# EvolEcolGroup/tidypopgen

Measured on AMD Instinct MI355X. Metric: SNP-genotypes/s (N x M) for IBS+KING+GRM+Fst+PCA; max |delta| vs CPU ref (cpu_baseline.parity), higher is better.
Workload: dtype fp4-e2m1 operands (exact integers, f32 accumulate) for the cross-products, the PCA Gram and the grouped counts, int8 (int32 accumulate) for the loadings, f64 for statistics

## Files before the change

### tidypopgen_amd/csrc/pca.hip

```cpp
#include <math.h>
#include <stdio.h>
#include <stdlib.h>
#include <string.h>
#include <time.h>

#include <algorithm>

#include "common.h"
#include <type_traits>
#include "devfrag.h"

#define MFMA_I8(a, b, c) __builtin_amdgcn_mfma_i32_32x32x32_i8((a), (b), (c), 0, 0, 0)
#define PCA_NAN __longlong_as_double(0x7FF8000000000000ll)

__global__ void tpg_pca_center_scale_kernel(const int4* __restrict__ counts, int64_t m, int64_t n,
                                            double* __restrict__ center, double* __restrict__ scale,
                                            int* __restrict__ flags) {
  for (int64_t j = blockIdx.x * (int64_t)blockDim.x + threadIdx.x; j < m; j += (int64_t)gridDim.x * blockDim.x) {
    const int4 c = counts[j];
    if (c.w != 0) flags[0] = 1;
    const double mean = (double)(c.y + 2 * c.z) / (double)n;
    const double p = mean / 2;
    const double sd = sqrt(2 * p * (1 - p));
    if (!(sd > 0)) flags[1] = 1;
// ... 1225 lines not shown
    std::vector<double> RR;
    if (first) {
      lam1 = fabs(theta[0]) > 0 ? fabs(theta[0]) : 1.0;
    } else {
      TPG_TRY(w.ritz(A, Y, act, X, theta, Y0, Y1, RR));
      TPG_HIP(tpg_copy_dev(ctx, A, Y0, colbytes(act)));
      if (nl == 0) lam1 = fabs(theta[0]) > 0 ? fabs(theta[0]) : 1.0;
      st.mark("ritz vectors + residuals");
    }
    int newly = 0;
    while (!first && newly < act && nl + newly < k && sqrt(std::max(0.0, RR[(size_t)newly])) < TOL * lam1) newly++;
    for (int j = 0; j < newly; j++) lam[(size_t)(nl + j)] = theta[(size_t)j];
    nl += newly;
    if (nl >= k) break;
    const int act2 = b - nl;
    TPG_REQUIRE(act2 >= 2, TPG_ENUMERIC, "eigen solver ran out of active vectors");
    double* A2 = Q + (size_t)n * nl;
    const double* KA2 = first ? Y : Y1 + (size_t)n * newly;
    const double up = std::max(theta[(size_t)act - 1], 1e-300 * lam1), lo = 0.0;
    const double a0 = std::max(theta[(size_t)newly], up * (1 + 1e-8));
    const double ec = (up - lo) / 2, cc = (up + lo) / 2;
    const double x0 = (a0 - cc) / ec;
    int deg = 20;
    if (x0 > 1.0 + 1e-12) {
      const double dmax = log(2 * AMP) / acosh(x0);
      deg = dmax < 2 ? 2 : (dmax > 20 ? 20 : (int)dmax);
    }
    if (tpg_env_set("TPG_DEBUG"))
      fprintf(stderr, "[eig] it %d act %d locked %d (+%d) deg %d theta_first %.4g theta_last %.4g lam1 %.4g res0 %.3g\n", it,
              act, nl, newly, deg, theta[(size_t)newly], theta[(size_t)act - 1], lam1,
              first ? -1.0 : sqrt(std::max(0.0, RR[(size_t)newly])) / lam1);
    w.b = act2;
    TPG_TRY(w.set_locked(Q, nl, lam.data()));
    double sigma = ec / (a0 - cc);
    const double sigma1 = sigma;
    double* prev = Y0;
    double* cur = first ? Y1 : Y;
    double* nxt = first ? Y : Y1;
    TPG_HIP(tpg_copy_dev(ctx, prev, A2, colbytes(act2)));
    TPG_LAUNCH(ctx, "eig_combine", tpg_combine_kernel, dim3(1024), dim3(256), 0, KA2, 1, (int64_t)n * act2,
               sigma1 / ec, (const double*)prev, -cc * sigma1 / ec, (const double*)nullptr, 0.0, cur,
               (const double*)nullptr);
    for (int dgr = 2; dgr <= deg; dgr++) {
      const double sigma2 = 1.0 / (2.0 / sigma1 - sigma);
      TPG_TRY(w.apply(cur, 2 * sigma2 / ec, cur, -2 * sigma2 * cc / ec, prev, -sigma * sigma2, nxt));
      double* t = prev; prev = cur; cur = nxt; nxt = t;
      sigma = sigma2;
    }
    TPG_HIP(tpg_copy_dev(ctx, A2, cur, colbytes(act2)));
    st.mark("chebyshev filter");
    TPG_TRY(orthonormalize(A2, act2, Q, nl, prev));
    st.mark("orthonormalize");
  }
  TPG_REQUIRE(nl >= k, TPG_ENUMERIC, "eigen solver did not converge (%d of %d pairs)", nl, k);
  for (int j = 0; j < k; j++) lambda_host[j] = lam[(size_t)j];
  TPG_HIP(tpg_copy_dev(ctx, d_U, Q, colbytes(k)));
  return TPG_OK;
}

static int pca_loadings_device(tpg_ctx* ctx, const tpg_view* v, const double* d_center, const double* d_scale,
                               const double* d_U, const double* d_dk, int k, double* d_V);

__global__ __launch_bounds__(256) void tpg_deflate_kernel(double* __restrict__ K, int n, const double* __restrict__ U,
                                                          const double* __restrict__ lam, int kb) {
  __shared__ double ui[16][33], uj[16][33];
  const int tx = threadIdx.x & 15, ty = threadIdx.x >> 4;
  const int i0 = blockIdx.x * 16, j0 = blockIdx.y * 16;
  for (int q = threadIdx.x; q < 16 * kb; q += 256) {
    const int r = q & 15, c = q >> 4;
    ui[r][c] = i0 + r < n ? U[(int64_t)(i0 + r) + (int64_t)c * n] * lam[c] : 0.0;
    uj[r][c] = j0 + r < n ? U[(int64_t)(j0 + r) + (int64_t)c * n] : 0.0;
  }
  __syncthreads();
  const int i = i0 + tx, j = j0 + ty;
  if (i >= n || j >= n) return;
  double s = 0.0;
  for (int c = 0; c < kb; c++) s = fma(ui[tx][c], uj[ty][c], s);
  K[(int64_t)i + (int64_t)j * n] -= s;
}

static int eig_topk_any(tpg_ctx* ctx, const double* d_K, int n, int k, double* lambda_host, double* d_U, double tol) {
  if (k <= 52) return eig_topk(ctx, d_K, n, k, lambda_host, d_U, tol);
  double *Kw = nullptr, *d_lam = nullptr;
  TPG_HIP(tpg_pmalloc((void**)&Kw, sizeof(double) * (size_t)n * (size_t)n));
  struct Free { void *a, *b; ~Free() { tpg_pfree(a); tpg_pfree(b); } } fr{Kw, nullptr};
  TPG_HIP(tpg_pmalloc((void**)&d_lam, sizeof(double) * 32));
  fr.b = d_lam;
  TPG_HIP(hipMemcpyAsync(Kw, d_K, sizeof(double) * (size_t)n * (size_t)n, hipMemcpyDeviceToDevice, ctx->stream));
  const int KB = 26;
  for (int done = 0; done < k;) {
    const int kb = std::min(KB, k - done);
    double* Ub = d_U + (size_t)done * (size_t)n;
    TPG_TRY(eig_topk(ctx, Kw, n, kb, lambda_host + done, Ub, tol));
    done += kb;
    if (done < k) {
      TPG_HIP(tpg_h2d_async(ctx, d_lam, lambda_host + done - kb, sizeof(double) * (size_t)kb));
      TPG_LAUNCH(ctx, "eig_deflate", tpg_deflate_kernel, dim3((unsigned)((n + 15) / 16), (unsigned)((n + 15) / 16)), dim3(256), 0, Kw, n,
                 (const double*)Ub, (const double*)d_lam, kb);
      TPG_CHECK_LAUNCH();
    }
  }
  return TPG_OK;
}

static int pca_svd_impl(tpg_ctx* ctx, tpg_comm* comm, const tpg_view* v, int k, double tol, double* d, double* u,
                        double* vload, double* center, double* scale, double* square_frobenius);

extern "C" int tpg_pca_partial_svd(tpg_ctx* ctx, const tpg_view* v, int k, double* d, double* u, double* vload,
                                   double* center, double* scale, double* square_frobenius) {
  TpgEnter _enter(ctx);
  return pca_svd_impl(ctx, nullptr, v, k, 1e-12, d, u, vload, center, scale, square_frobenius);
}

extern "C" int tpg_pca_partial_svd_sharded(tpg_ctx* ctx, tpg_comm* comm, const tpg_view* v, int k, double* d, double* u,
                                           double* vload, double* center, double* scale, double* square_frobenius) {
  TpgEnter _enter(ctx);
  TPG_REQUIRE(comm && comm->ctx == ctx, TPG_EINVAL, "bad communicator");
  return pca_svd_impl(ctx, comm, v, k, 1e-12, d, u, vload, center, scale, square_frobenius);
}

extern "C" int tpg_pca_random_svd(tpg_ctx* ctx, const tpg_view* v, int k, double tol, double* d, double* u,
                                  double* vload, double* center, double* scale, double* square_frobenius) {
  TpgEnter _enter(ctx);
  TPG_REQUIRE(tol > 0 && tol < 1, TPG_EINVAL, "tol = %g out of (0, 1)", tol);
  return pca_svd_impl(ctx, nullptr, v, k, tol < 1e-12 ? 1e-12 : tol, d, u, vload, center, scale, square_frobenius);
}

__global__ void tpg_tri_pack_kernel(const double* __restrict__ K, int n, double* __restrict__ tri) {
  const int64_t total = (int64_t)n * n;
  for (int64_t idx = blockIdx.x * (int64_t)blockDim.x + threadIdx.x; idx < total; idx += (int64_t)gridDim.x * blockDim.x) {
    const int64_t i = idx % n, k = idx / n;
    if (i <= k) tri[k * (k + 1) / 2 + i] = K[idx];
  }
}
__global__ void tpg_tri_unpack_kernel(const double* __restrict__ tri, int n, double* __restrict__ K) {
  const int64_t total = (int64_t)n * n;
  for (int64_t idx = blockIdx.x * (int64_t)blockDim.x + threadIdx.x; idx < total; idx += (int64_t)gridDim.x * blockDim.x) {
    const int64_t i = idx % n, k = idx / n;
    const int64_t lo = i < k ? i : k, hi = i < k ? k : i;
    K[idx] = tri[hi * (hi + 1) / 2 + lo];
  }
}

int tpg_pca_gram_allreduce(tpg_ctx* ctx, tpg_comm* comm, double* d_K, int64_t n) {
  if (!comm || !(comm->nranks > 1 || comm->nccl)) return TPG_OK;
  const int64_t ntri = n * (n + 1) / 2;
  double* d_tri = nullptr;
  hipError_t e = tpg_pmalloc((void**)&d_tri, sizeof(double) * (size_t)ntri);
  int lrc = TPG_OK;
  if (e != hipSuccess) { tpg_set_error("gram all-reduce: %s", hipGetErrorString(e)); (void)hipGetLastError(); lrc = TPG_EHIP; }
  lrc = tpg_comm_agree(comm, lrc);
  if (lrc != TPG_OK) { tpg_pfree(d_tri); return lrc; }
  TPG_LAUNCH(ctx, "pca_gram_tri", tpg_tri_pack_kernel, dim3(2048), dim3(256), 0, (const double*)d_K, (int)n, d_tri);
  int rc;
  {
    ProfScope ps(ctx, "pca_gram_allreduce");
    rc = tpg_comm_allreduce(comm, d_tri, ntri, 1);
  }
  if (rc == TPG_OK) TPG_LAUNCH(ctx, "pca_gram_tri", tpg_tri_unpack_kernel, dim3(2048), dim3(256), 0, (const double*)d_tri, (int)n, d_K);
  tpg_pfree(d_tri);
  return rc;
}

static int pca_svd_impl(tpg_ctx* ctx, tpg_comm* comm, const tpg_view* v, int k, double tol, double* d, double* u,
                        double* vload, double* center, double* scale, double* square_frobenius) {
  TPG_REQUIRE(ctx && v && d && u && vload && center && scale, TPG_EINVAL, "null argument");
  TPG_REQUIRE(k >= 1 && k <= v->n, TPG_EINVAL, "k = %d out of range", k);
  const int64_t n = v->n, m = v->m;
  OutBuf oc, os, ou, ov;
  int32_t* d_counts = nullptr;
  double *d_K = nullptr, *d_dk = nullptr, *d_tri = nullptr;
  struct Free { void *a, *b, *c, *d; ~Free() { tpg_pfree(a); tpg_pfree(b); tpg_pfree(c); tpg_pfree(d); } } fr{nullptr, nullptr, nullptr, nullptr};
  StageTimer st(ctx, "svd");
  const bool exchange = comm && (comm->nranks > 1 || comm->nccl);
  const int64_t ntri = n * (n + 1) / 2;
  auto local_steps = [&]() -> int {
    TPG_REQUIRE(k <= m, TPG_EINVAL, "k = %d but this view has %lld loci", k, (long long)m);
    TPG_TRY(oc.init(center, sizeof(double) * (size_t)m));
    TPG_TRY(os.init(scale, sizeof(double) * (size_t)m));
    TPG_TRY(ou.init(u, sizeof(double) * (size_t)n * (size_t)k));
    TPG_TRY(ov.init(vload, sizeof(double) * (size_t)m * (size_t)k));
    TPG_HIP(tpg_pmalloc((void**)&d_counts, sizeof(int32_t) * 4 * (size_t)m));
    fr.a = d_counts;
    TPG_HIP(tpg_pmalloc((void**)&d_K, sizeof(double) * (size_t)n * (size_t)n));
    fr.b = d_K;
    TPG_HIP(tpg_pmalloc((void**)&d_dk, sizeof(double) * (size_t)k));
    fr.d = d_dk;
    if (exchange) {
      TPG_HIP(tpg_pmalloc((void**)&d_tri, sizeof(double) * (size_t)ntri));
      fr.c = d_tri;
    }
    TPG_TRY(pca_counts_center_scale(ctx, v, d_counts, oc.dev<double>(), os.dev<double>()));
    st.mark("counts, center, scale");
    if (square_frobenius) TPG_TRY(frobenius_from_counts(ctx, v, d_counts, oc.dev<double>(), os.dev<double>(), square_frobenius));
    return TPG_OK;
  };
  int lrc = local_steps();
  if (exchange) lrc = tpg_comm_agree(comm, lrc);
  TPG_TRY(lrc);
  if (square_frobenius && exchange) TPG_TRY(tpg_comm_allreduce_f64(ctx, comm, square_frobenius, 1));
  st.mark("frobenius + alloc K");
  auto gram_branch = [&]() -> int {
    bool exchanged = false;
    if (exchange) TPG_TRY(tpg_gram_classes_exchanged(ctx, comm, v, d_counts, os.dev<double>(), d_K, &exchanged));
    if (exchanged) return pca_double_center_inplace(ctx, d_K, n);
    return pca_gram_device(ctx, v, oc.dev<double>(), os.dev<double>(), d_K, true);
  };
  int grc = gram_branch();
  if (exchange) grc = tpg_comm_agree(comm, grc);
  TPG_TRY(grc);
  st.mark("gram");
  if (exchange) {
    TPG_LAUNCH(ctx, "pca_gram_tri", tpg_tri_pack_kernel, dim3(2048), dim3(256), 0, (const double*)d_K, (int)n, d_tri);
    {
      ProfScope ps(ctx, "pca_gram_allreduce");
      TPG_TRY(tpg_comm_allreduce(comm, d_tri, ntri, 1));
    }
    TPG_LAUNCH(ctx, "pca_gram_tri", tpg_tri_unpack_kernel, dim3(2048), dim3(256), 0, (const double*)d_tri, (int)n, d_K);
  }
  std::vector<double> lam((size_t)k);
  TPG_TRY(eig_topk_any(ctx, d_K, (int)n, k, lam.data(), ou.dev<double>(), tol));
  st.mark("eig_topk");
  std::vector<double> dh((size_t)k);
  for (int j = 0; j < k; j++) dh[(size_t)j] = sqrt(lam[(size_t)j] > 0 ? lam[(size_t)j] : 0.0);
  TPG_HIP(tpg_push_small(ctx, d_dk, dh.data(), sizeof(double) * (size_t)k));
  TPG_TRY(pca_loadings_device(ctx, v, oc.dev<double>(), os.dev<double>(), ou.dev<double>(), d_dk, k, ov.dev<double>()));
  if (tpg_is_device_ptr(d)) TPG_HIP(tpg_push_small(ctx, d, dh.data(), sizeof(double) * (size_t)k));
  else memcpy(d, dh.data(), sizeof(double) * (size_t)k);
  TPG_HIP(hipStreamSynchronize(ctx->stream));
  st.mark("loadings");
  TPG_TRY(oc.commit(ctx));
  TPG_TRY(os.commit(ctx));
  TPG_TRY(ou.commit(ctx));
  return ov.commit(ctx);
}

#define LD_TU 6

__global__ void tpg_u_digits_kernel(const double* __restrict__ U, int64_t n, int k, int FU, int64_t Q, int CT,
                                    uint4* __restrict__ UD) {
  const int64_t total = Q * 4 * CT * 64;
  for (int64_t idx = blockIdx.x * (int64_t)blockDim.x + threadIdx.x; idx < total;
       idx += (int64_t)gridDim.x * blockDim.x) {
    const int lane = (int)(idx & 63);
    const int64_t tq = idx >> 6;
    const int ct = (int)(tq % CT);
    const int64_t qs = tq / CT;
    const int s = (int)(qs & 3);
    const int64_t q = qs >> 2;
    const int col = 32 * ct + (lane & 31), h = lane >> 5;
    const int kk = col / LD_TU, t = col % LD_TU;
    uint32_t w[4] = {0, 0, 0, 0};
    if (kk < k)
      for (int e = 0; e < 16; e++) {
        const int64_t i = 128 * q + 32 * s + 16 * h + e;
        if (i >= n) continue;
        long long W = llrint(ldexp(U[i + (int64_t)kk * n], FU));
        long long dig = 0;
        for (int tt = 0; tt <= t; tt++) {
          dig = W & 127;
          if (dig >= 64) dig -= 128;
          W = (W - dig) >> 7;
        }
        w[e >> 2] |= (uint32_t)((int)dig & 0xFF) << (8 * (e & 3));
      }
    UD[idx] = make_uint4(w[0], w[1], w[2], w[3]);
  }
}

__global__ __launch_bounds__(256) void tpg_uq_colsum_kernel(const double* __restrict__ U, int64_t n, int FU,
                                                            double* __restrict__ usum) {
  __shared__ double sh[256];
  const int kk = blockIdx.x;
  double acc = 0;
  for (int64_t i = threadIdx.x; i < n; i += 256) acc += ldexp((double)llrint(ldexp(U[i + (int64_t)kk * n], FU)), -FU);
  sh[threadIdx.x] = acc;
  __syncthreads();
  for (int w = 128; w > 0; w >>= 1) {
    if ((int)threadIdx.x < w) sh[threadIdx.x] += sh[threadIdx.x + w];
    __syncthreads();
  }
  if (threadIdx.x == 0) usum[kk] = sh[0];
}

#ifndef LD_NLT
#define LD_NLT 2
#endif
#ifndef LD_WGS
#define LD_WGS 2
#endif
__device__ __forceinline__ int64_t tpg_uniform64_pca(int64_t x) {
  const uint32_t lo = __builtin_amdgcn_readfirstlane((uint32_t)x), hi = __builtin_amdgcn_readfirstlane((uint32_t)((uint64_t)x >> 32));
  return (int64_t)(((uint64_t)hi << 32) | lo);
}

template <int C, class F>
__device__ __forceinline__ void tpg_pca_static_for(F&& f) {
  if constexpr (C > 0) {
    tpg_pca_static_for<C - 1>(f);
    f(std::integral_constant<int, C - 1>{});
  }
}

template <int CTP>
__global__ __launch_bounds__(256, LD_WGS) void tpg_loadings_mfma_kernel(const uint4* __restrict__ L,
                                                                   const uint4* __restrict__ UD, int64_t n_lt,
                                                                   int64_t Q, int ct0, int CT,
                                                                   int32_t* __restrict__ out, int Cpad) {
  __shared__ __attribute__((aligned(16))) uint4 ubuf[2][4 * CTP][64];
  const int lane = threadIdx.x & 63, wv = threadIdx.x >> 6;
  const int64_t lt0 = ((int64_t)blockIdx.x * 4 + wv) * LD_NLT;
  v16i acc[LD_NLT][CTP];
#pragma unroll
  for (int t = 0; t < LD_NLT; t++)
#pragma unroll
    for (int c = 0; c < CTP; c++)
#pragma unroll
      for (int r = 0; r < 16; r++) acc[t][c][r] = 0;
  const int Qi = (int)Q;
  const int64_t lt0u = tpg_uniform64_pca(lt0);
  const char* pa[LD_NLT];
#pragma unroll
  for (int t = 0; t < LD_NLT; t++) pa[t] = (const char*)(L + ((lt0u + t < n_lt ? lt0u + t : 0) * Q) * 64);
  auto LDG = [&](const char* p, int blk) {
    uint32_t off = (uint32_t)lane * 16u + (uint32_t)blk * 1024u;
    asm("" : "+v"(off));
    return *(const uint4*)(p + off);
  };
  constexpr int LD_D = 4;
  static_assert(LD_D % 2 == 0, "the slot of a group's digit fragments is its parity");
  uint4 AR[LD_D][LD_NLT];
#pragma unroll
  for (int d = 0; d < LD_D - 1; d++)
#pragma unroll
    for (int t = 0; t < LD_NLT; t++) AR[d][t] = LDG(pa[t], d < Qi ? d : Qi - 1);
  const char* pu = (const char*)(UD + ct0 * 64);
  uint4 un[2][CTP];
  auto ufrag = [&](int q, int j) {
    const int it = wv + 4 * j;
    return LDG(pu, (q * 4 + it / CTP) * CT + it % CTP);
  };
#pragma unroll
  for (int j = 0; j < CTP; j++) {
    ubuf[0][wv + 4 * j][lane] = ufrag(0, j);
    un[1][j] = ufrag(Qi > 1 ? 1 : 0, j);
  }
  tpg_lds_barrier();
  auto group = [&](auto Cc, auto Mm, int q) {
    constexpr int C = decltype(Cc)::value, M = decltype(Mm)::value;
    const int qa = q + LD_D - 1 < Qi ? q + LD_D - 1 : Qi - 1, qu = q + 2 < Qi ? q + 2 : Qi - 1;
    const int cur = q & 1;
#pragma unroll
    for (int t = 0; t < LD_NLT; t++) AR[M][t] = LDG(pa[t], qa);
#pragma unroll
    for (int j = 0; j < CTP; j++) un[C & 1][j] = ufrag(qu, j);
#pragma unroll
    for (int s = 0; s < 4; s++) {
      v4i fg[LD_NLT];
#pragma unroll
      for (int t = 0; t < LD_NLT; t++) {
        const uint32_t w = s == 0 ? AR[C][t].x : s == 1 ? AR[C][t].y : s == 2 ? AR[C][t].z : AR[C][t].w;
#pragma unroll
        for (int k = 0; k < 4; k++) fg[t][k] = (int)tpg_codes(w, k);
      }
#pragma unroll
      for (int c = 0; c < CTP; c++) {
        const uint4 bq = ubuf[cur][s * CTP + c][lane];
        v4i fb = {(int)bq.x, (int)bq.y, (int)bq.z, (int)bq.w};
#pragma unroll
        for (int t = 0; t < LD_NLT; t++) acc[t][c] = MFMA_I8(fg[t], fb, acc[t][c]);
      }
    }
#pragma unroll
    for (int j = 0; j < CTP; j++) ubuf[cur ^ 1][wv + 4 * j][lane] = un[(C & 1) ^ 1][j];
    tpg_lds_barrier();
  };
  for (int q = 0; q < Qi; q += LD_D)
    tpg_pca_static_for<LD_D>([&](auto kk) {
      constexpr int k = decltype(kk)::value;
      if (q + k < Qi) group(std::integral_constant<int, k>{}, std::integral_constant<int, (k + LD_D - 1) % LD_D>{}, q + k);
    });
#pragma unroll
  for (int t = 0; t < LD_NLT; t++) {
    if (lt0 + t >= n_lt) break;
#pragma unroll
    for (int c = 0; c < CTP; c++)
#pragma unroll
      for (int r = 0; r < 16; r++) {
        const int64_t row = (lt0 + t) * 32 + tpg_cd_row(r, lane);
        out[row * Cpad + 32 * (ct0 + c) + (lane & 31)] = acc[t][c][r];
      }
  }
}

__global__ void tpg_loadings_finalize_kernel(const int32_t* __restrict__ acc, int Cpad, int64_t m, int k, int FU,
                                             const double* __restrict__ center, const double* __restrict__ scale,
                                             const double* __restrict__ usum, const double* __restrict__ d,
                                             double* __restrict__ vload) {
  const int64_t total = m * k;
  for (int64_t idx = blockIdx.x * (int64_t)blockDim.x + threadIdx.x; idx < total;
       idx += (int64_t)gridDim.x * blockDim.x) {
    const int kk = (int)(idx % k);
    const int64_t j = idx / k;
    long long S = 0;
#pragma unroll
    for (int t = LD_TU - 1; t >= 0; t--) S = S * 128 + (long long)acc[j * Cpad + kk * LD_TU + t];
    const double gu = ldexp((double)S, -FU);
    vload[j + (int64_t)kk * m] = (gu - center[j] * usum[kk]) / (scale[j] * d[kk]);
  }
}

__global__ __launch_bounds__(1024) void tpg_absmax_kernel(const double* __restrict__ x, int64_t total, double* __restrict__ out) {
  __shared__ double sh[1024];
  double mx = 0;
  bool bad = false;
  for (int64_t i = threadIdx.x; i < total; i += 1024) {
    const double a = fabs(x[i]);
    if (a != a) bad = true;
    mx = a > mx ? a : mx;
  }
  sh[threadIdx.x] = bad ? __longlong_as_double(0x7FF8000000000000ll) : mx;
  __syncthreads();
  for (int w = 512; w > 0; w >>= 1) {
    if ((int)threadIdx.x < w) {
      const double a = sh[threadIdx.x], b = sh[threadIdx.x + w];
      sh[threadIdx.x] = (a != a || b != b) ? __longlong_as_double(0x7FF8000000000000ll) : (a > b ? a : b);
    }
    __syncthreads();
  }
  if (threadIdx.x == 0) out[0] = sh[0];
}

static int pca_loadings_device(tpg_ctx* ctx, const tpg_view* v, const double* d_center, const double* d_scale,
                               const double* d_U, const double* d_dk, int k, double* d_V) {
  const int64_t n = v->n, m = v->m;
  double amax = 0;
  {
    double* d_amax = nullptr;
    TPG_HIP(tpg_pmalloc((void**)&d_amax, sizeof(double)));
    TPG_LAUNCH(ctx, "loadings_u_digits", tpg_absmax_kernel, dim3(1), dim3(1024), 0, d_U, n * (int64_t)k, d_amax);
    hipError_t ea = tpg_fetch_small(ctx, &amax, d_amax, sizeof(double));
    tpg_pfree(d_amax);
    TPG_HIP(ea);
  }
  TPG_REQUIRE(amax > 0 && amax == amax && amax < 1e300, TPG_ENUMERIC, "degenerate eigenvectors");
  int ex = 0;
  frexp(amax, &ex);
  const int FU = 7 * LD_TU - 2 - ex;
  const int CT = (int)ceil_div((int64_t)k * LD_TU, 32);
  const int Cpad = CT * 32;
  const int64_t n_lt = v->KG * 4;
  uint4* d_UD = nullptr;
  int32_t* d_acc = nullptr;
  double* d_usum = nullptr;
  hipError_t e = tpg_pmalloc((void**)&d_UD, (size_t)v->Q * 4 * CT * 1024);
  if (e == hipSuccess) e = tpg_pmalloc((void**)&d_acc, sizeof(int32_t) * (size_t)n_lt * 32 * (size_t)Cpad);
  if (e == hipSuccess) e = tpg_pmalloc((void**)&d_usum, sizeof(double) * (size_t)k);
  if (e == hipSuccess) {
    TPG_LAUNCH(ctx, "loadings_u_digits", tpg_u_digits_kernel, dim3(1024), dim3(256), 0, d_U, n, k, FU, v->Q, CT, d_UD);
    TPG_LAUNCH(ctx, "loadings_u_digits", tpg_uq_colsum_kernel, dim3((unsigned)k), dim3(256), 0, d_U, n, FU, d_usum);
    const unsigned grid = (unsigned)ceil_div(n_lt, 4 * LD_NLT);
    for (int ct0 = 0; ct0 < CT;) {
      const int left = CT - ct0;
#define LD_LAUNCH(C)                                                                                             \
  TPG_LAUNCH(ctx, "loadings_mfma", tpg_loadings_mfma_kernel<C>, dim3(grid), dim3(256), 0, (const uint4*)v->L,     \
             (const uint4*)d_UD, n_lt, v->Q, ct0, CT, d_acc, Cpad)
      if (left >= 4) { LD_LAUNCH(4); ct0 += 4; }
      else if (left == 3) { LD_LAUNCH(3); ct0 += 3; }
      else if (left == 2) { LD_LAUNCH(2); ct0 += 2; }
      else { LD_LAUNCH(1); ct0 += 1; }
#undef LD_LAUNCH
    }
    TPG_LAUNCH(ctx, "loadings_finalize", tpg_loadings_finalize_kernel, dim3(2048), dim3(256), 0, (const int32_t*)d_acc,
               Cpad, m, k, FU, d_center, d_scale, (const double*)d_usum, d_dk, d_V);
    e = hipGetLastError();
    if (e == hipSuccess) e = hipStreamSynchronize(ctx->stream);
  }
  tpg_pfree(d_UD); tpg_pfree(d_acc); tpg_pfree(d_usum);
  if (e != hipSuccess) { tpg_set_error("loadings: %s", hipGetErrorString(e)); return TPG_EHIP; }
  return TPG_OK;
}

int tpg_sym_eig_topk_tol(tpg_ctx* ctx, const double* d_K, int64_t n, int k, double tol, double* lambda_host, double* d_U) {
  TPG_REQUIRE(ctx && d_K && lambda_host && d_U, TPG_EINVAL, "null argument");
  TPG_REQUIRE(n > 0 && k >= 1 && k <= n, TPG_EINVAL, "bad n = %lld / k = %d", (long long)n, k);
  return eig_topk_any(ctx, d_K, (int)n, k, lambda_host, d_U, tol);
}

extern "C" int tpg_sym_eig_topk(tpg_ctx* ctx, const double* K, int64_t n, int k, double* lambda, double* U) {
  TpgEnter _enter(ctx);
  TPG_REQUIRE(ctx && K && lambda && U, TPG_EINVAL, "null argument");
  TPG_REQUIRE(n > 0 && k >= 1 && k <= n, TPG_EINVAL, "bad n = %lld / k = %d", (long long)n, k);
  InBuf ik;
  TPG_TRY(ik.init(ctx, K, sizeof(double) * (size_t)n * (size_t)n));
  OutBuf ou;
  TPG_TRY(ou.init(U, sizeof(double) * (size_t)n * (size_t)k));
  std::vector<double> lam((size_t)k);
  TPG_TRY(eig_topk_any(ctx, ik.dev<double>(), (int)n, k, lam.data(), ou.dev<double>(), 1e-12));
  if (tpg_is_device_ptr(lambda)) TPG_HIP(hipMemcpyAsync(lambda, lam.data(), sizeof(double) * (size_t)k, hipMemcpyHostToDevice, ctx->stream));
  else memcpy(lambda, lam.data(), sizeof(double) * (size_t)k);
  TPG_HIP(hipStreamSynchronize(ctx->stream));
  return ou.commit(ctx);
}

extern "C" int tpg_pca_loadings(tpg_ctx* ctx, const tpg_view* v, const double* center, const double* scale,
                                const double* U, const double* d, int k, double* vload) {
  TpgEnter _enter(ctx);
  TPG_REQUIRE(ctx && v && center && scale && U && d && vload, TPG_EINVAL, "null argument");
  TPG_REQUIRE(k >= 1, TPG_EINVAL, "k must be positive");
  const int64_t n = v->n, m = v->m;
  InBuf ic, is, iu, id;
  TPG_TRY(ic.init(ctx, center, sizeof(double) * (size_t)m));
  TPG_TRY(is.init(ctx, scale, sizeof(double) * (size_t)m));
  TPG_TRY(iu.init(ctx, U, sizeof(double) * (size_t)n * (size_t)k));
  TPG_TRY(id.init(ctx, d, sizeof(double) * (size_t)k));
  OutBuf ov;
  TPG_TRY(ov.init(vload, sizeof(double) * (size_t)m * (size_t)k));
  int32_t* d_counts = nullptr;
  int* d_flag = nullptr;
  TPG_HIP(tpg_pmalloc((void**)&d_counts, sizeof(int32_t) * 4 * (size_t)m));
  hipError_t e = tpg_pmalloc((void**)&d_flag, 2 * sizeof(int));
  int flag[2] = {0, 1};
  int rc = e == hipSuccess ? tpg_launch_loci_counts(ctx, v, d_counts) : TPG_EHIP;
  if (rc == TPG_OK) {
    e = hipMemsetAsync(d_flag, 0, 2 * sizeof(int), ctx->stream);
    TPG_LAUNCH(ctx, "pca_center_check", tpg_center_is_mean_kernel, dim3(1024), dim3(256), 0, (const int4*)d_counts,
               ic.dev<double>(), m, n, d_flag);
    if (e == hipSuccess) e = tpg_fetch_small(ctx, flag, d_flag, 2 * sizeof(int));
    if (e != hipSuccess) { tpg_set_error("pca_loadings: %s", hipGetErrorString(e)); rc = TPG_EHIP; }
  }
  tpg_pfree(d_counts);
  tpg_pfree(d_flag);
  TPG_TRY(rc);
  if (!flag[1]) {
    rc = pca_loadings_device(ctx, v, ic.dev<double>(), is.dev<double>(), iu.dev<double>(), id.dev<double>(), k,
                             ov.dev<double>());
  } else {
    double* d_inv = nullptr;
    TPG_HIP(tpg_pmalloc((void**)&d_inv, sizeof(double) * (size_t)m));
    TPG_LAUNCH(ctx, "inv_scale", tpg_inv_kernel, dim3(1024), dim3(256), 0, is.dev<double>(), m, d_inv);
    rc = run_sweep(ctx, SW_ROWSCALE, v->L, v->KG * 4, v->Q, m, n, ic.dev<double>(), d_inv, iu.dev<double>(), n, k,
                   ov.dev<double>(), id.dev<double>(), nullptr);
    tpg_pfree(d_inv);
  }
  TPG_TRY(rc);
  return ov.commit(ctx);
}
```

Measured before the change: 134.8 billion.

## Fuse loadings finalize into MFMA epilogue and parallelize absmax reduction

When all column tiles fit in one launch (CT<=4), the loadings MFMA kernel now stages its int32 accumulators through LDS per wave and directly reconstructs the digit sums and writes the final double loadings. This skips the int32 accumulator buffer round-trip and the separate finalize kernel. The absmax over U becomes a two-stage multi-workgroup reduction instead of a single 1024-thread block. The risks are LDS reuse hazards, since the staging area aliases the U buffers, and a less coalesced, strided loading write pattern in the epilogue.

```diff
diff --git a/tidypopgen_amd/csrc/pca.hip b/tidypopgen_amd/csrc/pca.hip
--- a/tidypopgen_amd/csrc/pca.hip
+++ b/tidypopgen_amd/csrc/pca.hip
@@ -1551,12 +1551,27 @@
   }
 }
 
-template <int CTP>
+__device__ __forceinline__ double tpg_loading_value(long long S, int FU, double center, double scale, double usum, double d) {
+  const double gu = ldexp((double)S, -FU);
+  return (gu - center * usum) / (scale * d);
+}
+
+struct LdFin {
+  int64_t m;
+  int k, FU;
+  const double *center, *scale, *usum, *d;
+  double* vload;
+};
+
+template <int CTP, bool FUSE>
 __global__ __launch_bounds__(256, LD_WGS) void tpg_loadings_mfma_kernel(const uint4* __restrict__ L,
                                                                    const uint4* __restrict__ UD, int64_t n_lt,
                                                                    int64_t Q, int ct0, int CT,
-                                                                   int32_t* __restrict__ out, int Cpad) {
-  __shared__ __attribute__((aligned(16))) uint4 ubuf[2][4 * CTP][64];
+                                                                   int32_t* __restrict__ out, int Cpad, LdFin fin) {
+  constexpr int LD_RS = 32 * CTP + 4;
+  __shared__ __attribute__((aligned(16))) uint4 ubuf_raw[2 * 4 * CTP * 64 + (FUSE ? 64 : 0)];
+  static_assert(!FUSE || 4 * 16 * LD_RS * sizeof(int32_t) <= sizeof(ubuf_raw), "staging slices");
+  uint4(*ubuf)[4 * CTP][64] = reinterpret_cast<uint4(*)[4 * CTP][64]>(ubuf_raw);
   const int lane = threadIdx.x & 63, wv = threadIdx.x >> 6;
   const int64_t lt0 = ((int64_t)blockIdx.x * 4 + wv) * LD_NLT;
   v16i acc[LD_NLT][CTP];
@@ -1629,16 +1644,56 @@
       constexpr int k = decltype(kk)::value;
       if (q + k < Qi) group(std::integral_constant<int, k>{}, std::integral_constant<int, (k + LD_D - 1) % LD_D>{}, q + k);
     });
-#pragma unroll
-  for (int t = 0; t < LD_NLT; t++) {
-    if (lt0 + t >= n_lt) break;
-#pragma unroll
-    for (int c = 0; c < CTP; c++)
-#pragma unroll
-      for (int r = 0; r < 16; r++) {
-        const int64_t row = (lt0 + t) * 32 + tpg_cd_row(r, lane);
-        out[row * Cpad + 32 * (ct0 + c) + (lane & 31)] = acc[t][c][r];
+  if constexpr (FUSE) {
+    int32_t* stage = reinterpret_cast<int32_t*>(ubuf_raw) + wv * (16 * LD_RS);
+    const int row = lane & 15;
+#pragma unroll
+    for (int t = 0; t < LD_NLT; t++) {
+      if (lt0 + t >= n_lt) break;
+#pragma unroll
+      for (int p = 0; p < 2; p++) {
+#pragma unroll
+        for (int c = 0; c < CTP; c++)
+#pragma unroll
+          for (int rr = 0; rr < 8; rr++)
+            stage[((rr & 3) + 8 * (rr >> 2) + 4 * (lane >> 5)) * LD_RS + 32 * c + (lane & 31)] = acc[t][c][8 * p + rr];
+        __builtin_amdgcn_fence(__ATOMIC_RELEASE, "wavefront");
+        __builtin_amdgcn_wave_barrier();
+        __builtin_amdgcn_fence(__ATOMIC_ACQUIRE, "wavefront");
+        const int64_t j = (lt0 + t) * 32 + 16 * p + row;
+        if (j < fin.m) {
+          const double cj = fin.center[j], sj = fin.scale[j];
+          for (int kk = lane >> 4; kk < fin.k; kk += 4) {
+            const int2* dg = reinterpret_cast<const int2*>(stage + row * LD_RS + kk * LD_TU);
+            static_assert(LD_TU == 6, "three 8-byte reads per component");
+            const int2 d01 = dg[0], d23 = dg[1], d45 = dg[2];
+            long long S = 0;
+            S = S * 128 + (long long)d45.y;
+            S = S * 128 + (long long)d45.x;
+            S = S * 128 + (long long)d23.y;
+            S = S * 128 + (long long)d23.x;
+            S = S * 128 + (long long)d01.y;
+            S = S * 128 + (long long)d01.x;
+            fin.vload[j + (int64_t)kk * fin.m] = tpg_loading_value(S, fin.FU, cj, sj, fin.usum[kk], fin.d[kk]);
+          }
+        }
+        __builtin_amdgcn_fence(__ATOMIC_RELEASE, "wavefront");
+        __builtin_amdgcn_wave_barrier();
+        __builtin_amdgcn_fence(__ATOMIC_ACQUIRE, "wavefront");
       }
+    }
+  } else {
+#pragma unroll
+    for (int t = 0; t < LD_NLT; t++) {
+      if (lt0 + t >= n_lt) break;
+#pragma unroll
+      for (int c = 0; c < CTP; c++)
+#pragma unroll
+        for (int r = 0; r < 16; r++) {
+          const int64_t row = (lt0 + t) * 32 + tpg_cd_row(r, lane);
+          out[row * Cpad + 32 * (ct0 + c) + (lane & 31)] = acc[t][c][r];
+        }
+    }
   }
 }
 
@@ -1654,16 +1709,16 @@
     long long S = 0;
 #pragma unroll
     for (int t = LD_TU - 1; t >= 0; t--) S = S * 128 + (long long)acc[j * Cpad + kk * LD_TU + t];
-    const double gu = ldexp((double)S, -FU);
-    vload[j + (int64_t)kk * m] = (gu - center[j] * usum[kk]) / (scale[j] * d[kk]);
-  }
-}
-
+    vload[j + (int64_t)kk * m] = tpg_loading_value(S, FU, center[j], scale[j], usum[kk], d[kk]);
+  }
+}
+
+#define LD_AMAX_WGS 64
 __global__ __launch_bounds__(1024) void tpg_absmax_kernel(const double* __restrict__ x, int64_t total, double* __restrict__ out) {
   __shared__ double sh[1024];
   double mx = 0;
   bool bad = false;
-  for (int64_t i = threadIdx.x; i < total; i += 1024) {
+  for (int64_t i = blockIdx.x * (int64_t)1024 + threadIdx.x; i < total; i += (int64_t)gridDim.x * 1024) {
     const double a = fabs(x[i]);
     if (a != a) bad = true;
     mx = a > mx ? a : mx;
@@ -1677,7 +1732,7 @@
     }
     __syncthreads();
   }
-  if (threadIdx.x == 0) out[0] = sh[0];
+  if (threadIdx.x == 0) out[blockIdx.x] = sh[0];
 }
 
 static int pca_loadings_device(tpg_ctx* ctx, const tpg_view* v, const double* d_center, const double* d_scale,
@@ -1686,8 +1741,10 @@
   double amax = 0;
   {
     double* d_amax = nullptr;
-    TPG_HIP(tpg_pmalloc((void**)&d_amax, sizeof(double)));
-    TPG_LAUNCH(ctx, "loadings_u_digits", tpg_absmax_kernel, dim3(1), dim3(1024), 0, d_U, n * (int64_t)k, d_amax);
+    TPG_HIP(tpg_pmalloc((void**)&d_amax, sizeof(double) * (LD_AMAX_WGS + 1)));
+    const int wgs = (int)std::min<int64_t>(LD_AMAX_WGS, ceil_div(n * (int64_t)k, 1024));
+    TPG_LAUNCH(ctx, "loadings_u_digits", tpg_absmax_kernel, dim3(wgs), dim3(1024), 0, d_U, n * (int64_t)k, d_amax + 1);
+    TPG_LAUNCH(ctx, "loadings_u_digits", tpg_absmax_kernel, dim3(1), dim3(1024), 0, (const double*)(d_amax + 1), (int64_t)wgs, d_amax);
     hipError_t ea = tpg_fetch_small(ctx, &amax, d_amax, sizeof(double));
     tpg_pfree(d_amax);
     TPG_HIP(ea);
@@ -1699,29 +1756,38 @@
   const int CT = (int)ceil_div((int64_t)k * LD_TU, 32);
   const int Cpad = CT * 32;
   const int64_t n_lt = v->KG * 4;
+  const bool fuse = CT <= 4;
   uint4* d_UD = nullptr;
   int32_t* d_acc = nullptr;
   double* d_usum = nullptr;
   hipError_t e = tpg_pmalloc((void**)&d_UD, (size_t)v->Q * 4 * CT * 1024);
-  if (e == hipSuccess) e = tpg_pmalloc((void**)&d_acc, sizeof(int32_t) * (size_t)n_lt * 32 * (size_t)Cpad);
+  if (e == hipSuccess && !fuse) e = tpg_pmalloc((void**)&d_acc, sizeof(int32_t) * (size_t)n_lt * 32 * (size_t)Cpad);
   if (e == hipSuccess) e = tpg_pmalloc((void**)&d_usum, sizeof(double) * (size_t)k);
   if (e == hipSuccess) {
     TPG_LAUNCH(ctx, "loadings_u_digits", tpg_u_digits_kernel, dim3(1024), dim3(256), 0, d_U, n, k, FU, v->Q, CT, d_UD);
     TPG_LAUNCH(ctx, "loadings_u_digits", tpg_uq_colsum_kernel, dim3((unsigned)k), dim3(256), 0, d_U, n, FU, d_usum);
     const unsigned grid = (unsigned)ceil_div(n_lt, 4 * LD_NLT);
-    for (int ct0 = 0; ct0 < CT;) {
-      const int left = CT - ct0;
-#define LD_LAUNCH(C)                                                                                             \
-  TPG_LAUNCH(ctx, "loadings_mfma", tpg_loadings_mfma_kernel<C>, dim3(grid), dim3(256), 0, (const uint4*)v->L,     \
-             (const uint4*)d_UD, n_lt, v->Q, ct0, CT, d_acc, Cpad)
-      if (left >= 4) { LD_LAUNCH(4); ct0 += 4; }
-      else if (left == 3) { LD_LAUNCH(3); ct0 += 3; }
-      else if (left == 2) { LD_LAUNCH(2); ct0 += 2; }
-      else { LD_LAUNCH(1); ct0 += 1; }
+    const LdFin fin{m, k, FU, d_center, d_scale, d_usum, d_dk, d_V};
+#define LD_LAUNCH(C, F, ct0)                                                                                       \
+  TPG_LAUNCH(ctx, "loadings_mfma", (tpg_loadings_mfma_kernel<C, F>), dim3(grid), dim3(256), 0, (const uint4*)v->L, \
+             (const uint4*)d_UD, n_lt, v->Q, ct0, CT, d_acc, Cpad, fin)
+    if (fuse) {
+      if (CT == 4) LD_LAUNCH(4, true, 0);
+      else if (CT == 3) LD_LAUNCH(3, true, 0);
+      else if (CT == 2) LD_LAUNCH(2, true, 0);
+      else LD_LAUNCH(1, true, 0);
+    } else {
+      for (int ct0 = 0; ct0 < CT;) {
+        const int left = CT - ct0;
+        if (left >= 4) { LD_LAUNCH(4, false, ct0); ct0 += 4; }
+        else if (left == 3) { LD_LAUNCH(3, false, ct0); ct0 += 3; }
+        else if (left == 2) { LD_LAUNCH(2, false, ct0); ct0 += 2; }
+        else { LD_LAUNCH(1, false, ct0); ct0 += 1; }
+      }
+      TPG_LAUNCH(ctx, "loadings_finalize", tpg_loadings_finalize_kernel, dim3(2048), dim3(256), 0, (const int32_t*)d_acc,
+                 Cpad, m, k, FU, d_center, d_scale, (const double*)d_usum, d_dk, d_V);
+    }
 #undef LD_LAUNCH
-    }
-    TPG_LAUNCH(ctx, "loadings_finalize", tpg_loadings_finalize_kernel, dim3(2048), dim3(256), 0, (const int32_t*)d_acc,
-               Cpad, m, k, FU, d_center, d_scale, (const double*)d_usum, d_dk, d_V);
     e = hipGetLastError();
     if (e == hipSuccess) e = hipStreamSynchronize(ctx->stream);
   }
```

Result: no change. 135.4 billion, median of 6 (+0.5%).
